# wthanone/kmerLSH

Hardware: AMD Instinct MI355X
Metric: k-mers·iterations/sec (LSH+cluster loop), 10M k-mers × 64 samples (higher is better)
Workload: dtype f32

## Files before the change

### kmerlsh_amd/csrc/klsh_ctx.h

```cpp
#pragma once
#include <hip/hip_runtime.h>
#include <stdint.h>
#include <stdio.h>
#include <string.h>

#include <atomic>
#include <chrono>
#include <cmath>
#include <string>
#include <thread>
#include <utility>
#include <vector>

#include "klsh.h"
#include "klsh_comm.h"
#include "klsh_internal.h"

extern "C" void klsh_host_hyperplanes(uint32_t base, uint64_t k0, uint64_t count, int d,
                                      int stride, float* out, int threads);

namespace klsh {

int fail(int code, const std::string& msg);
inline int set_error(int code, const char* msg) { return fail(code, msg); }
// ... 154 lines not shown
  uint32_t* pub_seq_dev = nullptr;
  uint32_t pub_seq = 0;
  static constexpr int kRing = 2 * 32;
  Counters* ring_host = nullptr;
  Counters* ring_dev = nullptr;
  bool ctr_clean = false;
  uint32_t* n_next_dev = nullptr;
  klsh::QueuedProjection spec;
  bool take_queued_projection() {
    const bool queued = spec.pending;
    if (queued && spec.swap) std::swap(keys, keys2);
    drop_queued_projection();
    return queued;
  }
  void drop_queued_projection() { spec.pending = spec.swap = false; }
  bool zero_copy = true;
  klsh::RunCounters* rc = nullptr;
  uint16_t* xh_alloc = nullptr;
  bool shadow_wanted(int d_) const {
    return pw.variant != klsh::kProjPacked && klsh::shadow_width_ok(d_);
  }
  bool tail_batch = true;
  bool tail_local = true;
  int last_hash_kernel = klsh::kPkNone;
  int last_hash_variant = klsh::kPvNone;
  uint64_t last_hash_close = 0;
  bool result_device = false;
  uint32_t result_rounds = 0;
  int64_t result_rank_us = 0;
  klsh::KmcHooks kmc;
  klsh::KcountHooks kcount;

  ~klsh_ctx() { release(); }

  bool phase_timing = false;

  uint64_t shard_min_rows = 1u << 21;
  uint32_t huge_quiet = 0;
  bool huge_fold_always = false;
  double comm_timeout_s = 600.0;

  int stop_after = 0;
  hipEvent_t counts_ev = nullptr;
  int progress = 0;
  void tick(int it) const {
    if (progress > 0 && it % progress == 0) {
// ... 37 lines not shown
```

### kmerlsh_amd/csrc/klsh_device.h

```cpp
#pragma once
#include <hip/hip_runtime.h>

#include "klsh_internal.h"

namespace klsh {
__device__ __forceinline__ unsigned long long stamp_now() { return __builtin_amdgcn_s_memrealtime(); }
__device__ __forceinline__ void kt_begin(const KTime& kt, int c) {
  if (kt.blk && threadIdx.x == 0) {
    const unsigned long long now = stamp_now();
    atomicMin(&kt.blk->set[kt.set].t0[c][blockIdx.x % kStampSlots].v, now);
    if (kt.phase >= 0) atomicMin(&kt.blk->set[kt.set].t0[kt.phase][blockIdx.x % kStampSlots].v, now);
  }
}
__device__ __forceinline__ void kt_end(const KTime& kt, int c) {
  if (kt.blk && threadIdx.x == 0) {
    const unsigned long long now = stamp_now();
    atomicMax(&kt.blk->set[kt.set].t1[c][blockIdx.x % kStampSlots].v, now);
    if (kt.phase >= 0) atomicMax(&kt.blk->set[kt.set].t1[kt.phase][blockIdx.x % kStampSlots].v, now);
  }
}
__device__ __forceinline__ void kt_fold_set(KStampBlock* blk, int f, uint32_t t) {
  if (t >= (uint32_t)KC_COUNT) return;
  KStampSet& st = blk->set[f];
  unsigned long long lo = ~0ull, hi = 0ull;
  for (int q = 0; q < kStampSlots; ++q) {
    lo = min(lo, __hip_atomic_load(&st.t0[t][q].v, __ATOMIC_RELAXED, __HIP_MEMORY_SCOPE_AGENT));
    hi = max(hi, __hip_atomic_load(&st.t1[t][q].v, __ATOMIC_RELAXED, __HIP_MEMORY_SCOPE_AGENT));
    __hip_atomic_store(&st.t0[t][q].v, ~0ull, __ATOMIC_RELAXED, __HIP_MEMORY_SCOPE_AGENT);
    __hip_atomic_store(&st.t1[t][q].v, 0ull, __ATOMIC_RELAXED, __HIP_MEMORY_SCOPE_AGENT);
  }
  if (hi != 0ull && lo != ~0ull && hi >= lo) {
// ... 362 lines not shown
```

### kmerlsh_amd/csrc/klsh_internal.h

```cpp
#pragma once

#include <hip/hip_ext.h>
#include <hip/hip_runtime_api.h>
#include <stdint.h>
#include <stdio.h>

#include <vector>

#include "klsh.h"

namespace klsh {

constexpr uint32_t kInvalid = 0xFFFFFFFFu;
constexpr uint32_t kNil = 0xFFFFFFFFu;
constexpr int kMaxHyperplanes = 32;
constexpr int kScanTile = 4096;
uint64_t sort_ws_words(uint64_t slots);
constexpr uint32_t kScanStatusWord = 64;
constexpr uint64_t kScanSumsWord = kScanStatusWord + 2ull * (1ull << 20);
inline uint64_t scan_ws_words(uint64_t slots) {
  return kScanSumsWord + (256 * slots) / kScanTile + 1024;
}

constexpr int kBigClasses = 4;
// ... 35 lines not shown
  KC_TAIL, KC_COMPACT, KC_SCREEN,
  KC_MERGE,
  KC_COUNT
};
constexpr int kStampSlots = 16;
struct alignas(128) StampLine {
  unsigned long long v;
  unsigned long long pad_[15];
};
struct KStampSet {
  StampLine t0[KC_COUNT][kStampSlots];
  StampLine t1[KC_COUNT][kStampSlots];
};
struct KStampBlock {
  KStampSet set[2];
  unsigned long long ticks[KC_COUNT];
  unsigned long long launches[KC_COUNT];
};
struct KTime {
  KStampBlock* blk;
  int set;
  int fold;
  int phase = -1;
};
constexpr KTime kNoTime{nullptr, 0, -1, -1};

struct MergeWork {
  uint2* cls[kGroupClasses];
  uint2* act[kGroupClasses];
  uint32_t screened;
  uint2* big[kBigClasses];
  uint2* huge;
  uint2* over;
  uint32_t* tile_sums;
  RunCounters* rc;
  uint32_t* run_ws;
  uint32_t* dlist;
  uint32_t* mark;
  uint32_t stamp;
  uint32_t big896_aux;
  uint32_t huge_cap;
  uint32_t huge_fold;
  uint64_t* long_P;
  uint32_t long_groups;
  uint32_t long_off = 4;
  uint32_t small_grid;
// ... 88 lines not shown

const uint32_t* radix_sort_top(const uint32_t* k0, const uint32_t* v0, uint32_t* k1, uint32_t* v1,
                               uint32_t n, int bits, uint32_t* ws, hipStream_t s, KTime kt,
                               const uint32_t* n_dev);
void launch_tail_local(const uint32_t* kin, const uint32_t* vin, uint32_t* kout, uint32_t* vout,
                       const uint32_t* dtot, int bits, int bucket_thr, const MergeWork& w,
                       hipStream_t s);
constexpr int kTailTopBits = 9;
constexpr int kTailLowBits = 19 - kTailTopBits > 10 ? 19 - kTailTopBits : 10;
inline bool tail_local_ok(uint32_t n_max, int bits) {
  return n_max <= (1u << 20) && bits > kTailTopBits && bits <= kTailTopBits + kTailLowBits;
}

constexpr int kRunListCount = kGroupClasses + kBigClasses + 2;
void launch_runs(const uint32_t* key, uint32_t lo, uint32_t n, int bucket_thr, const MergeWork& w,
                 hipStream_t s, const uint32_t* n_dev = nullptr);

struct Publish {
  Counters* host;
  uint32_t* seq_host;
  uint32_t seq;
  uint32_t* n_next;
  uint32_t* woff = nullptr;
};

struct LookBack {
  unsigned long long* status;
  mutable uint32_t epoch;
};

void launch_compact(const uint32_t* slots, uint32_t n, uint32_t* out, uint32_t* tile_sums,
                    Counters* ctr, hipStream_t s, const Publish* pub = nullptr,
                    RunCounters* rc = nullptr, KTime kt = kNoTime,
                    const LookBack* lb = nullptr, const uint32_t* n_dev = nullptr);
void launch_stamp_fold(KStampBlock* blk, int set, hipStream_t s);
void launch_publish_words(const uint32_t* a, uint32_t na, const uint32_t* b, uint32_t nb,
                          uint32_t* dst, uint32_t* seq_host, uint32_t seq, hipStream_t s);

void launch_convert(const Rows& r, const uint16_t* counts, uint32_t bs, const float* lut,
                    const float* v_kmers, uint32_t* keep, uint32_t* order, uint32_t* tile_sums,
                    Counters* ctr, hipStream_t s);

void launch_norms(const Rows& r, uint32_t n, hipStream_t s);
void launch_shadow_build(const Rows& r, uint64_t n, hipStream_t s);


// ... 149 lines not shown
```

### kmerlsh_amd/csrc/klsh_kernels.hip

```cpp
#include <hip/hip_runtime.h>

#include <stdlib.h>

#include <string>
#include <type_traits>

#include "klsh_device.h"

namespace klsh {

typedef float f32x2 __attribute__((ext_vector_type(2)));


__device__ __forceinline__ void pk_mac_lo(f32x2& acc, f32x2 w, f32x2 x) {
  f32x2 t;
  asm("v_pk_mul_f32 %1, %2, %3 op_sel_hi:[1,0]\n\tv_pk_add_f32 %0, %0, %1"
      : "+v"(acc), "=&v"(t) : "v"(w), "v"(x));
}
__device__ __forceinline__ void pk_mac_hi(f32x2& acc, f32x2 w, f32x2 x) {
  f32x2 t;
  asm("v_pk_mul_f32 %1, %2, %3 op_sel:[0,1] op_sel_hi:[1,1]\n\tv_pk_add_f32 %0, %0, %1"
      : "+v"(acc), "=&v"(t) : "v"(w), "v"(x));
}

// ... 849 lines not shown
    case 64: go_pk(k_project_pk<64, 2, 1>); break;
    default: {
      const size_t lds = sizeof(float4) * (size_t)r.dp * (size_t)((h + 3) / 4);
      if (lds <= 64 * 1024) {
        static const bool lds_ok =
            hipFuncSetAttribute(reinterpret_cast<const void*>(&k_project_wide_pk<1>),
                                hipFuncAttributeMaxDynamicSharedMemorySize, 64 * 1024) == hipSuccess;
        (void)lds_ok;
        k_project_wide_pk<1><<<grid, block, lds, s>>>(r.x, r.d, r.dp, slots, keys, n, W, h, key_or,
                                                      kt);
        pv = kPvWidePk;
      } else {
        pv = kPvGeneric;
        k_project_generic<<<grid, block, 0, s>>>(r.x, r.d, r.dp, slots, keys, n, W, h, key_or, kt);
      }
    }
  }
  return kPkPacked;
}

constexpr int kCompactTile = 4096;
__global__ __launch_bounds__(256) void k_compact_count(const uint32_t* __restrict__ slots,
                                                       uint32_t n, uint32_t* __restrict__ counts,
                                                       KTime kt) {
  __shared__ uint32_t wsum[4];
  kt_begin(kt, KC_COMPACT);
  const uint32_t t = threadIdx.x, lane = t & 63u, wv = t >> 6;
  const uint32_t T0 = blockIdx.x * (uint32_t)kCompactTile;
  uint32_t c = 0;
#pragma unroll
  for (int k = 0; k < kCompactTile / 256; ++k) {
    const uint32_t i = T0 + k * 256u + t;
    const uint32_t v = slots[i < n ? i : 0u];
    c += (uint32_t)__popcll(__ballot(i < n && v != kInvalid));
  }
  if (lane == 0) wsum[wv] = c;
  __syncthreads();
  if (t == 0) counts[blockIdx.x] = wsum[0] + wsum[1] + wsum[2] + wsum[3];
}

__device__ __forceinline__ void collect_run_counts(Counters* ctr, RunCounters* rc) {
  if (!rc) return;
  ctr->n_seg = rc->n_seg.v;
  rc->n_seg.v = 0u;
#pragma unroll
  for (int c = 0; c < kGroupClasses; ++c) {
    ctr->n_cls[c] = rc->n_cls[c].v;
    rc->n_cls[c].v = 0u;
  }
#pragma unroll
// ... 6 lines not shown
  ctr->n_over = rc->n_over.v;
  rc->n_over.v = 0u;
  ctr->n_small_rows = rc->n_small_rows.v;
  rc->n_small_rows.v = 0u;
#pragma unroll
  for (int c = 0; c < kBigClasses; ++c) {
    ctr->n_big_rows[c] = rc->n_big_rows[c].v;
    rc->n_big_rows[c].v = 0u;
  }
  ctr->n_huge_rows = rc->n_huge_rows.v;
  rc->n_huge_rows.v = 0u;
#pragma unroll
  for (int c = 0; c < kGroupClasses; ++c) rc->n_act[c].v = 0u;
  ctr->n_act_rows = rc->n_act_rows.v;
  rc->n_act_rows.v = 0u;
  ctr->screened = rc->screened.v;
  rc->screened.v = 0u;
}

__device__ __forceinline__ void publish_counters(Counters* ctr, uint32_t total, const Publish& pub,
                                                 uint32_t n_in) {
  Counters c = *ctr;
  c.total = total;
  if (pub.n_next) *pub.n_next = total;
  if (pub.woff && n_in) *pub.woff += 31u - (uint32_t)__builtin_clz(n_in);
  const uint32_t* src = reinterpret_cast<const uint32_t*>(&c);
  uint32_t* dst = reinterpret_cast<uint32_t*>(pub.host);
  for (int i = 0; i < (int)(sizeof(Counters) / 4); ++i) {
    __hip_atomic_store(dst + i, src[i], __ATOMIC_RELAXED, __HIP_MEMORY_SCOPE_SYSTEM);
    reinterpret_cast<uint32_t*>(ctr)[i] = 0u;
  }
  __threadfence_system();
  __hip_atomic_store(pub.seq_host, pub.seq, __ATOMIC_RELEASE, __HIP_MEMORY_SCOPE_SYSTEM);
}

__global__ void k_publish(Counters* ctr, Publish pub, RunCounters* rc) {
  collect_run_counts(ctr, rc);
  if (pub.host) publish_counters(ctr, ctr->total, pub, 0u);
}

__global__ __launch_bounds__(256) void k_compact_apply(const uint32_t* __restrict__ slots,
                                                       uint32_t n,
                                                       const uint32_t* __restrict__ counts,
                                                       uint32_t* __restrict__ out,
                                                       uint32_t* __restrict__ total,
                                                       Counters* ctr, Publish pub,
                                                       RunCounters* rc, KTime kt) {
  constexpr int K = kCompactTile / 256;
  __shared__ uint32_t cnt[K * 4], pre[K * 4 + 1], wsum[4];
  const uint32_t t = threadIdx.x, lane = t & 63u, wv = t >> 6;
  const uint32_t T0 = blockIdx.x * (uint32_t)kCompactTile;
  uint32_t before = 0;
  for (uint32_t j = t; j < blockIdx.x; j += 256) before += counts[j];
#pragma unroll
  for (int o = 32; o > 0; o >>= 1) before += __shfl_xor(before, o, 64);
  if (lane == 0) wsum[wv] = before;
  uint32_t v[K];
  uint64_t m[K];
#pragma unroll
  for (int k = 0; k < K; ++k) {
    const uint32_t i = T0 + k * 256u + t;
    v[k] = slots[i < n ? i : 0u];
  }
#pragma unroll
  for (int k = 0; k < K; ++k) {
    if (T0 + k * 256u + t >= n) v[k] = kInvalid;
    m[k] = __ballot(v[k] != kInvalid);
    if (lane == 0) cnt[k * 4 + wv] = (uint32_t)__popcll(m[k]);
  }
  __syncthreads();
  if (t == 0) {
    uint32_t a = wsum[0] + wsum[1] + wsum[2] + wsum[3];
    for (int q = 0; q < K * 4; ++q) {
// ... 74 lines not shown
      a += cnt[q];
    }
    pre[K * 4] = a;
  }
  __syncthreads();
  const uint64_t below = lane ? (~0ull >> (64 - lane)) : 0ull;
#pragma unroll
  for (int k = 0; k < K; ++k)
    if (v[k] != kInvalid) out[pre[k * 4 + wv] + (uint32_t)__popcll(m[k] & below)] = v[k];
  if (blockIdx.x == gridDim.x - 1 && t == 0) {
    *total = pre[K * 4];
    collect_run_counts(ctr, rc);
    if (pub.host) publish_counters(ctr, pre[K * 4], pub, n);
  }
  kt_end(kt, KC_COMPACT);
}

void launch_compact(const uint32_t* slots, uint32_t n, uint32_t* out, uint32_t* tile_sums,
                    Counters* ctr, hipStream_t s, const Publish* pub, RunCounters* rc, KTime kt,
                    const LookBack* lb, const uint32_t* n_dev) {
  const Publish none{nullptr, nullptr, 0u, nullptr};
  if (n_dev) {
    const uint32_t ntiles = (n + kCompactTile - 1) / kCompactTile;
    if (!lb || !lb->status || ntiles == 0 || ntiles > 256u) return;
    const uint32_t epoch = ++lb->epoch;
    k_compact_lb<<<ntiles, 256, 0, s>>>(slots, n, out, lb->status, epoch, &ctr->total, ctr,
                                        pub ? *pub : none, rc, kt, n_dev);
    return;
  }
  if (n == 0) {
    (void)hipMemsetAsync(&ctr->total, 0, sizeof(uint32_t), s);
    k_publish<<<1, 1, 0, s>>>(ctr, pub ? *pub : none, rc);
    return;
  }
  const uint32_t ntiles = (n + kCompactTile - 1) / kCompactTile;
  if (lb && lb->status && ntiles <= 256u) {
    const uint32_t epoch = ++lb->epoch;
    k_compact_lb<<<ntiles, 256, 0, s>>>(slots, n, out, lb->status, epoch, &ctr->total, ctr,
                                        pub ? *pub : none, rc, kt, nullptr);
    return;
  }
  uint32_t* counts = tile_sums + kScanSumsWord;
  k_compact_count<<<ntiles, 256, 0, s>>>(slots, n, counts, kt);
  k_compact_apply<<<ntiles, 256, 0, s>>>(slots, n, counts, out, &ctr->total, ctr, pub ? *pub : none,
                                         rc, kt);
}

__global__ __launch_bounds__(256) void k_convert(Rows r, const uint16_t* __restrict__ counts,
                                                 uint32_t bs, const float* __restrict__ lut,
                                                 const float* __restrict__ v_kmers,
                                                 uint32_t* __restrict__ keep) {
  const uint32_t i = blockIdx.x * 256u + threadIdx.x;
  if (i >= bs) return;
  const int d = r.d;
  float* x = r.x + (size_t)i * r.dp;
  uint64_t total = 0;
  float nn = 0.0f;
  for (int j = 0; j < d; ++j) {
    const uint32_t c = counts[(size_t)j * bs + i];
    total += c;
    const float v = lut[c] - v_kmers[j];
    x[j] = v;
    nn = nn + v * v;
  }
  for (int j = d; j < r.dp; ++j) x[j] = 0.0f;
  r.nrm[i] = nn;
  r.cnt[i] = 1;
  r.head[i] = i;
// ... 77 lines not shown
```

### kmerlsh_amd/csrc/klsh_loop.cpp

```cpp
#include <stddef.h>
#include <stdlib.h>
#include <string.h>

#include <algorithm>
#include <deque>

#include "klsh_loop.h"

namespace klsh {

static void count_class_rows(klsh_stats* st, const Counters& c, uint64_t n, bool tail) {
  uint64_t big_rows = 0, big_runs = 0, small_runs = 0;
  for (int b = 0; b < kBigClasses; ++b) big_rows += c.n_big_rows[b], big_runs += c.n_big[b];
  for (int b = 0; b < kGroupClasses; ++b) small_runs += c.n_cls[b];
  for (int k : {KC_PROJECT, KC_SORT, KC_COMPACT}) st->kern[k].rows += n;
  st->kern[KC_RUNS].rows += n;
  st->kern[KC_RUNS].runs += c.n_seg;
  st->kern[KC_HUGE].rows += c.n_huge_rows;
  st->kern[KC_HUGE].runs += c.n_huge;
  if (c.screened) {
    st->kern[KC_SCREEN].rows += c.n_small_rows;
    st->kern[KC_SCREEN].runs += small_runs;
  }
  const uint64_t merged_small = c.screened ? c.n_act_rows : c.n_small_rows;
// ... 167 lines not shown
    const uint64_t k = *rng_counter;
    *rng_counter += (uint64_t)h2;
    if (st) {
      st->hyperplanes += (uint64_t)h2;
      st->nested_calls += 1;
    }
    if (int e = ctx->ensure_hyperplanes(seed_base, k, (uint64_t)h2, st ? &st->host_ms : nullptr))
      return e;
    const uint32_t key_or = 0x80000000u | ((oi & 1u) << 30);
    launch_project(ctx->rows, fv + p, ctx->nk1, b, ctx->hyperplane_ptr(k), h2, key_or, s, &ctx->pw);
    uint32_t *rk = nullptr, *rv = nullptr;
    radix_sort(ctx->nk1, fv + p, ctx->nk2, ctx->nv2, b, h2, ctx->hist, &rk, &rv, s);
    KLSH_HIP(hipMemcpyAsync(fk + p, rk, 4ull * b, hipMemcpyDeviceToDevice, s));
    if (rv != fv + p) KLSH_HIP(hipMemcpyAsync(fv + p, rv, 4ull * b, hipMemcpyDeviceToDevice, s));
    KLSH_HIP(hipMemsetAsync(ctx->rc, 0, sizeof(RunCounters), s));
    launch_merge(ctx->rows, fk, fv, p, p + b, thr, -1, ctx->mw, ctx->ctr, s);
    KLSH_HIP(hipGetLastError());
  }
  launch_compact(fv, n, out, ctx->tile_sums, ctx->ctr, s, nullptr, ctx->rc);
  KLSH_HIP(hipGetLastError());
  return ctx->sync_counters();
}

int merge_and_compact(klsh_ctx* ctx, uint32_t* fk, uint32_t* fv, uint32_t n, float thr,
                      int bucket_thr, uint32_t seed_base, uint64_t* rng_counter, klsh_stats* st,
                      bool timed, const std::function<int(uint32_t*)>* after, KTime kt) {
  uint32_t* out = (fv == ctx->order) ? ctx->alt : ctx->order;
  if (int e = merge_main(ctx, fk, fv, n, thr, bucket_thr, out, st, timed, true, after, kt))
    return e;
  ctx->mw.big896_aux = ctx->h_ctr->n_big[kBigClasses - 1] >= 64u ? 1u : 0u;
  ctx->mw.huge_cap = ctx->h_ctr->n_huge == 0 ? 64u : 0u;
  ctx->huge_quiet = ctx->h_ctr->n_huge == 0 ? ctx->huge_quiet + 1 : 0;
  ctx->mw.huge_fold = (ctx->huge_quiet >= 4 || ctx->huge_fold_always) ? 1u : 0u;
  if (ctx->h_ctr->n_over > 0) {
    std::vector<uint2> over;
    uint64_t hyp = 0;
    if (int e = oversize_runs(ctx, &over, &hyp)) return e;
    if (int e = merge_nested(ctx, fk, fv, n, thr, over, seed_base, rng_counter, out, st))
      return e;
  }
  if (out == ctx->alt) std::swap(ctx->order, ctx->alt);
  ctx->n_live = ctx->h_ctr->total;
  return 0;
}

static bool batch_eligible(const klsh_ctx* ctx, uint64_t n, int bucket_thr, int iters_left) {
  if (!ctx->tail_batch || n < 2 || n >= std::min<uint64_t>(tail_merge_max(ctx->mw), 1u << 20) ||
      iters_left < 2)
    return false;
  if (bucket_thr >= 0 && n > (uint64_t)bucket_thr) return false;
  if (!ctx->zero_copy || !ctx->ring_dev || !ctx->lb.status || ctx->phase_timing) return false;
  if (!project_device_n_ok(ctx->d) || ctx->mw.dlist) return false;
  if (diag_host_driven()) return false;
  return (uint64_t)iters_left * (uint64_t)floor_log2(n) * (uint64_t)ctx->dp <= (64ull << 20);
}

static int run_batched(klsh_ctx* ctx, float& threshold, float sim_step, int it, int it_end,
                       int bucket_size_threshold, uint32_t seed_base, uint64_t* rng_counter,
                       uint64_t* nt_trace, klsh_stats* st,
                       const std::function<KTime(uint64_t)>& ktime) {
  hipStream_t s = ctx->stream;
#ifdef KLSH_MERGE_PROF
  if (getenv("KLSH_MERGE_PROF")) {
    fprintf(stderr, "[mprof] ---- head: iterations before %d\n", it);
    merge_prof_dump(stderr);
    fprintf(stderr, "[mprof] ---- tail: iterations %d..%d\n", it, it_end - 1);
  }
#endif
  constexpr int C = klsh_ctx::kRing / 2;
  uint64_t n_known = ctx->n_live;
  const int h0 = floor_log2(n_known);
  const uint64_t k0 = *rng_counter;
  const uint64_t need = (uint64_t)(it_end - it) * (uint64_t)h0;
  if (!(ctx->W && ctx->w_base == seed_base && ctx->w_dp == ctx->dp && ctx->w_d == ctx->d &&
        k0 >= ctx->w_k0 && k0 + need <= ctx->w_k0 + ctx->w_count)) {
    if (!ctx->lazy_covers(seed_base, k0, need)) KLSH_HIP(hipStreamSynchronize(s));
    if (int e = ctx->ensure_hyperplanes(seed_base, k0, need, &st->host_ms)) return e;
  }
  uint32_t* n_dev = ctx->n_next_dev;
  uint32_t* woff_dev = ctx->n_next_dev + 1;
  KLSH_HIP(hipMemsetD32Async(n_dev, (int)(uint32_t)n_known, 1, s));
  KLSH_HIP(hipMemsetD32Async(woff_dev, (int)(uint32_t)(k0 - ctx->w_k0), 1, s));
  const uint64_t queued_k = ctx->spec.k;
  bool queued = ctx->take_queued_projection();
  if (!queued && !ctx->ctr_clean)
    if (int e = ctx->reset_counters()) return e;
  if (queued && queued_k != k0) return fail(KLSH_E_STATE, "queued projection out of step");

  struct Chunk {
    int it0, count, slot0;
    uint32_t seq_last;
  };
  std::deque<Chunk> inflight;
  int next = it, slot = 0;
  float thr = threshold;
  uint64_t n_max = n_known;
  auto enqueue = [&](int count) -> int {
    const int hb = floor_log2(n_max);
    for (int c = 0; c < count; ++c, ++next) {
      const KTime kt = ktime(ctx->kt_iter++);
      if (!queued)
        launch_project_device_n(ctx->rows, ctx->order, ctx->keys, (uint32_t)n_max, ctx->W, n_dev, s,
                                kt, woff_dev, &ctx->pw);
      queued = false;
      uint32_t *fk = nullptr, *fv = nullptr;
      const bool local = ctx->tail_local && tail_local_ok((uint32_t)n_max, hb);
      LaunchScope launch(ctx->mw, kt);
      if (local) {
        const uint32_t* dtot = radix_sort_top(ctx->keys, ctx->order, ctx->keys2, ctx->alt,
                                              (uint32_t)n_max, hb, ctx->hist, s, kt, n_dev);
        launch_tail_local(ctx->keys2, ctx->alt, ctx->keys, ctx->order, dtot, hb,
                          bucket_size_threshold, ctx->mw, s);
        fk = ctx->keys;
        fv = ctx->order;
      } else {
        radix_sort(ctx->keys, ctx->order, ctx->keys2, ctx->alt, (uint32_t)n_max, hb, ctx->hist,
                   &fk, &fv, s, kt, n_dev);
      }
      launch_merge(ctx->rows, fk, fv, 0, (uint32_t)n_max, thr, bucket_size_threshold, ctx->mw,
                   ctx->ctr, s, n_dev, local);
      uint32_t* out = (fv == ctx->order) ? ctx->alt : ctx->order;
      Publish pub{ctx->ring_dev + slot, ctx->pub_seq_dev, ++ctx->pub_seq, n_dev, woff_dev};
      launch_compact(fv, (uint32_t)n_max, out, ctx->tile_sums, ctx->ctr, s, &pub, ctx->rc, kt,
                     &ctx->lb, n_dev);
      if (out == ctx->alt) std::swap(ctx->order, ctx->alt);
      thr -= sim_step;
      slot = (slot + 1) % klsh_ctx::kRing;
    }
    KLSH_HIP(hipGetLastError());
    return 0;
  };
  while (next < it_end || !inflight.empty()) {
    while (next < it_end && inflight.size() < 2) {
      const Chunk ch{next, std::min(C, it_end - next), slot, 0u};
      if (int e = enqueue(ch.count)) return e;
      inflight.push_back(ch);
      inflight.back().seq_last = ctx->pub_seq;
    }
    const Chunk ch = inflight.front();
    inflight.pop_front();
    if (int e = ctx->wait_seq(ch.seq_last)) return e;
    for (int c = 0; c < ch.count; ++c) {
      const Counters cc = ctx->ring_host[(ch.slot0 + c) % klsh_ctx::kRing];
      const uint64_t n_in = n_known;
      if (cc.err)
        return fail(KLSH_E_HIP, "device protocol failure (look-back wait limit), code " +
                                    std::to_string(cc.err));
      if (cc.n_over || n_in == 0 || cc.total == 0 || cc.total > n_in)
        return fail(KLSH_E_STATE, "queued iteration published inconsistent counters");
      const int h = floor_log2(n_in);
      if (nt_trace) nt_trace[ch.it0 + c] = n_in;
      ctx->tick(ch.it0 + c);
      *rng_counter += (uint64_t)h;
      account_iteration(st, n_in, h, cc.total);
      if (ctx->kernel_timing && ctx->kstamp) count_class_rows(st, cc, n_in, true);
      diag_log_batched(ch.it0 + c, n_in, h, cc);
      *ctx->h_ctr = cc;
      n_known = cc.total;
    }
    n_max = n_known;
  }
  threshold = thr;
  ctx->n_live = n_known;
  ctx->ctr_clean = true;
  return 0;
}

int run_single(klsh_ctx* ctx, float& threshold, float sim_step, int it_begin, int it_end,
               int bucket_size_threshold, uint32_t seed_base, uint64_t* rng_counter,
               uint64_t* nt_trace, klsh_stats* st) {
  hipStream_t s = ctx->stream;
  const uint64_t kt_first = ctx->kt_iter;
  auto ktime = [&](uint64_t j) -> KTime {
    if (!ctx->kernel_timing || !st) return kNoTime;
    if (!ctx->kstamp) return kNoTime;
    return KTime{ctx->kstamp, (int)(j & 1u), j > kt_first ? (int)((j - 1) & 1u) : -1};
  };
  for (int it = it_begin; it < it_end; ++it) {
    const uint64_t n = ctx->n_live;
    if (batch_eligible(ctx, n, bucket_size_threshold, it_end - it)) {
      const std::function<KTime(uint64_t)> kt_fn = ktime;
      if (int e = run_batched(ctx, threshold, sim_step, it, it_end, bucket_size_threshold,
                              seed_base, rng_counter, nt_trace, st, kt_fn))
        return e;
      break;
    }
    const double t_it = diag_iter_begin();
    if (nt_trace) nt_trace[it] = n;
    ctx->tick(it);
    if (n == 0) {
      account_iteration(st, 0, 0, 0);
      threshold -= sim_step;
      continue;
    }
    const int h = floor_log2(n);
    const uint64_t k = *rng_counter;
    *rng_counter += (uint64_t)h;
    if (int e = ctx->ensure_hyperplanes(seed_base, k, (uint64_t)h, &st->host_ms)) return e;

    const QueuedProjection spec = ctx->spec;
    const bool queued = ctx->take_queued_projection();
    const uint64_t j = ctx->kt_iter++;
    if (queued && spec.k != k) return fail(KLSH_E_STATE, "queued projection out of step");
    const int pair = queued ? spec.pair : 0;
    const bool rec = ctx->hip_events || ctx->phase_timing;
    if (!queued) {
      if (!ctx->ctr_clean) if (int e = ctx->reset_counters()) return e;
      if (rec) KLSH_HIP(hipEventRecord(ctx->project_begin(pair), s));
      launch_project(ctx->rows, ctx->order, ctx->keys, (uint32_t)n, ctx->hyperplane_ptr(k), h, 0u,
// ... 24 lines not shown
      ctx->spec = QueuedProjection{true, k_next, next_pair, spec_out == ctx->keys2};
      return 0;
    };
    if (int e = merge_and_compact(ctx, fk, fv, (uint32_t)n, threshold, bucket_size_threshold,
                                  seed_base, rng_counter, st, ctx->phase_timing,
                                  ahead ? &queue_next : nullptr, ktime(j)))
      return e;
    if (ctx->spec.pending && *rng_counter != ctx->spec.k) {
      ctx->drop_queued_projection();
      if (ctx->kernel_timing && ctx->kstamp) {
        KStampSet* set = &ctx->kstamp->set[ctx->kt_iter & 1u];
        KLSH_HIP(hipMemsetAsync(&set->t0[KC_PROJECT][0], 0xFF, sizeof(set->t0[KC_PROJECT]), s));
        KLSH_HIP(hipMemsetAsync(&set->t1[KC_PROJECT][0], 0, sizeof(set->t1[KC_PROJECT]), s));
      }
    }
    if (rec) {
      st->project_ms += elapsed(ctx->project_begin(pair), ctx->project_end(pair));
      st->project_timed_launches += 1;
    }
    if (rec && ctx->phase_timing)
      st->sort_ms += elapsed(ctx->project_end(pair), ctx->ev[EV_SORT_END]);
    account_iteration(st, n, h, ctx->n_live);
    threshold -= sim_step;
    diag_log_iteration(ctx, it, n, h, t_it);
  }
  if (ctx->kernel_timing && ctx->kstamp && st && ctx->kt_iter > kt_first)
    if (int e = collect_kernel_times(ctx, (int)((ctx->kt_iter - 1) & 1u), st)) return e;
  return 0;
}

}

using namespace klsh;

extern "C" int klsh_cluster(klsh_ctx* ctx, float min_similarity, int iterations,
                            int bucket_size_threshold, uint32_t seed_base, uint64_t* rng_counter,
                            uint64_t* nt_trace, klsh_stats* stats) {
  if (!ctx || !rng_counter) return fail(KLSH_E_ARG, "null argument");
  if (!ctx->loaded) {
    if (ctx->comm) ctx->comm->abort();
    return fail(KLSH_E_STATE, "klsh_cluster before a load");
  }
  KLSH_HIP(hipSetDevice(ctx->device));
  if (stats && stats->struct_size != sizeof(klsh_stats))
    return fail(KLSH_E_ARG, "klsh_stats.struct_size != sizeof(klsh_stats): built against another "
                            "klsh.h (KLSH_ABI_VERSION " + std::to_string(KLSH_ABI_VERSION) + ")");
  klsh_stats local{};
  klsh_stats* st = stats ? stats : &local;
  memset(st, 0, sizeof(*st));
  st->struct_size = sizeof(*st);
  st->world = (uint64_t)ctx->world();
  ctx->mw.huge_cap = 0;
  ctx->mw.huge_fold = ctx->huge_fold_always ? 1u : 0u;
  ctx->huge_quiet = 0;
  const int run_iters = ctx->stop_after > 0 ? std::min(iterations, ctx->stop_after) : iterations;
  if (ctx->comm)
    return cluster_sharded(ctx, min_similarity, iterations, run_iters, bucket_size_threshold,
                           seed_base, rng_counter, nt_trace, st);
  const double t_start = now_ms();

  const float max_similarity = 0.95f;
  const float sim_step = (max_similarity - min_similarity) / (float)iterations;
  float threshold = max_similarity;

  ctx->ctr_clean = false;
  ctx->drop_queued_projection();
  ctx->mw.big896_aux = ctx->n_live >= (1u << 24) ? 1u : 0u;
  ctx->w_count = 0;
  if (ctx->n_live > 0 && iterations > 0) {
    if (int e = ctx->predraw_hyperplanes(seed_base, *rng_counter,
                                         (uint64_t)floor_log2(ctx->n_live), iterations,
                                         &st->host_ms))
      return e;
  }

  if (int e = run_single(ctx, threshold, sim_step, 0, run_iters, bucket_size_threshold, seed_base,
                         rng_counter, nt_trace, st))
// ... 17 lines not shown
```

### kmerlsh_amd/csrc/klsh_loop.h

```cpp
#pragma once
#include <functional>
#include <vector>

#include "klsh_ctx.h"

namespace klsh {

struct LaunchScope {
  MergeWork& mw;
  LaunchScope(MergeWork& w, KTime kt, hipEvent_t e0 = nullptr, hipEvent_t e1 = nullptr) : mw(w) {
    mw.kt = kt, mw.small_ev[0] = e0, mw.small_ev[1] = e1;
  }
  ~LaunchScope() { mw.kt = kNoTime, mw.small_ev[0] = mw.small_ev[1] = nullptr; }
  LaunchScope(const LaunchScope&) = delete;
};

struct DeltaScope {
  MergeWork& mw;
  DeltaScope(MergeWork& w, uint32_t* dlist, uint32_t* mark, uint32_t stamp) : mw(w) {
    mw.dlist = dlist, mw.mark = mark, mw.stamp = stamp;
  }
  ~DeltaScope() { mw.dlist = mw.mark = nullptr; }
  DeltaScope(const DeltaScope&) = delete;
};

inline void account_iteration(klsh_stats* st, uint64_t n, int h, uint64_t n_next) {
  st->iterations += 1;
  if (n == 0) return;
  st->hyperplanes += (uint64_t)h;
  st->project_launches += 1;
  st->sum_rows += n;
  st->sum_proj_bits += n * (uint64_t)h;
  st->sum_merges += n - n_next;
}

int merge_main(klsh_ctx* ctx, uint32_t* fk, uint32_t* fv, uint32_t n, float thr, int bucket_thr,
               uint32_t* out, klsh_stats* st, bool timed, bool sync = true,
               const std::function<int(uint32_t*)>* after = nullptr, KTime kt = kNoTime);
int oversize_runs(klsh_ctx* ctx, std::vector<uint2>* over, uint64_t* hyperplanes);
int merge_nested(klsh_ctx* ctx, uint32_t* fk, uint32_t* fv, uint32_t n, float thr,
                 const std::vector<uint2>& over, uint32_t seed_base, uint64_t* rng_counter,
                 uint32_t* out, klsh_stats* st);
int merge_and_compact(klsh_ctx* ctx, uint32_t* fk, uint32_t* fv, uint32_t n, float thr,
                      int bucket_thr, uint32_t seed_base, uint64_t* rng_counter, klsh_stats* st,
                      bool timed, const std::function<int(uint32_t*)>* after = nullptr,
                      KTime kt = kNoTime);
int run_single(klsh_ctx* ctx, float& threshold, float sim_step, int it_begin, int it_end,
               int bucket_size_threshold, uint32_t seed_base, uint64_t* rng_counter,
               uint64_t* nt_trace, klsh_stats* st);
int cluster_sharded(klsh_ctx* ctx, float min_similarity, int iterations, int run_iters,
                    int bucket_size_threshold, uint32_t seed_base, uint64_t* rng_counter,
                    uint64_t* nt_trace, klsh_stats* st);

}
```

### kmerlsh_amd/csrc/klsh_merge.hip

```cpp
#include <algorithm>
#include <cstdlib>
#include <cstring>
#include <limits>

#include "klsh_merge_common.h"
#include "klsh_merge_small.h"
#include "klsh_merge_runs.h"
#include "klsh_merge_gram.h"
#include "klsh_merge_huge.h"
#include "klsh_merge_big.h"
#include "klsh_merge_long.h"
#include "klsh_merge_wide.h"

namespace klsh {

static float sim_roundtrip(float s) {
  volatile float dist = 1.0f - s;
  volatile float sim = 1.0f - dist;
  return sim;
}
static uint32_t ordered(float f) {
  uint32_t u;
  memcpy(&u, &f, 4);
  return (u & 0x80000000u) ? ~u : (u | 0x80000000u);
// ... 234 lines not shown
  else group(k_merge_group_wide<32>, 4, 2, dc);
  if (gram && gmin <= 16) group(k_merge_group_wide<16, 512>, 3, 4, dg);
  else group(k_merge_group_wide<16>, 3, 4, dc);
  if (gram && gmin <= 8) group(k_merge_group_wide<8, 512>, 2, 8, dg);
  else group(k_merge_group_wide<8>, 2, 8, dc);
  group(k_merge_group_wide<4>, 1, 16, dc);
  group(k_merge_group_wide<2>, 0, 32, dc);
}

void launch_runs(const uint32_t* key, uint32_t lo, uint32_t n, int bucket_thr, const MergeWork& w,
                 hipStream_t s, const uint32_t* n_dev) {
  const uint32_t ntiles = (n + kRunTile - 1) / kRunTile;
  uint32_t* counts = w.run_ws;
  uint32_t* tail_ends = counts + (size_t)kRunRows * ntiles;
  uint2* heads_fl = reinterpret_cast<uint2*>(counts + (((kRunRows + 1u) * ntiles + 1u) & ~1u));
  uint64_t* hbits = reinterpret_cast<uint64_t*>(heads_fl + ntiles);
  k_runs_count<<<ntiles, 256, 0, s>>>(key, lo, n, bucket_thr, ntiles, hbits, heads_fl, counts,
                                      w.kt, n_dev);
  const bool fused = ntiles <= 256u;
  if (fused) {
    k_runs_write<true><<<ntiles, 256, 0, s>>>(lo, n, bucket_thr, ntiles, hbits, heads_fl,
                                              tail_ends, counts, w, n_dev);
  } else {
    k_runs_scan<<<kRunRows, 256, 0, s>>>(counts, ntiles, n, bucket_thr, heads_fl, tail_ends, w.rc);
    k_runs_write<false><<<ntiles, 256, 0, s>>>(lo, n, bucket_thr, ntiles, hbits, heads_fl,
                                               tail_ends, counts, w, nullptr);
  }
}

void launch_tail_local(const uint32_t* kin, const uint32_t* vin, uint32_t* kout, uint32_t* vout,
                       const uint32_t* dtot, int bits, int bucket_thr, const MergeWork& w,
                       hipStream_t s) {
  k_tail_local<<<1u << kTailTopBits, 256, 0, s>>>(kin, vin, kout, vout, dtot, bits - kTailTopBits,
                                                   bucket_thr, w);
}

void launch_merge(const Rows& r, const uint32_t* key, uint32_t* slots, uint32_t lo, uint32_t hi,
                  float thr, int bucket_thr, const MergeWork& w, Counters* ctr, hipStream_t s,
                  const uint32_t* n_dev, bool runs_ready) {
  if (hi <= lo) return;
  const uint32_t n = hi - lo;
  if (n_dev && (lo != 0 || n >= tail_merge_max(w))) return;
  const Decider dc = make_decider(thr);
  if (!runs_ready) launch_runs(key, lo, n, bucket_thr, w, s, n_dev);
  MergeWork wm = w;
  if (w.kt.blk && (n >= tail_merge_max(w) || !project_device_n_ok(r.d))) wm.kt.phase = KC_MERGE;
  switch (r.d) {
// ... 64 lines not shown
```

### kmerlsh_amd/csrc/klsh_merge_runs.h

```cpp
#pragma once

#include "klsh_merge_common.h"

namespace klsh {

constexpr uint32_t kRunTile = 4096;
constexpr int kRunLists = kGroupClasses + kBigClasses + 2;
constexpr int kRunRows = kRunLists + 2 + kBigClasses + 1;

__device__ __forceinline__ uint32_t* run_counter(RunCounters* rc, int l) {
  return l < kGroupClasses ? &rc->n_cls[l].v
         : l < kGroupClasses + kBigClasses ? &rc->n_big[l - kGroupClasses].v
         : l == kRunLists - 2 ? &rc->n_huge.v
         : l == kRunLists - 1 ? &rc->n_over.v
         : l == kRunLists ? &rc->n_seg.v
         : l == kRunLists + 1 ? &rc->n_small_rows.v
         : l < kRunLists + 2 + kBigClasses ? &rc->n_big_rows[l - kRunLists - 2].v
                                           : &rc->n_huge_rows.v;
}

__device__ __forceinline__ int run_class(uint32_t b, int bucket_thr) {
  if (bucket_thr >= 0 && b > (uint32_t)bucket_thr) return kRunLists - 1;
  if (b > 64u) {
    if (b > (uint32_t)kBigRows[kBigClasses - 1]) return kRunLists - 2;
// ... 136 lines not shown
  for (int o = 32; o > 0; o >>= 1) {
    heads += __shfl_xor(heads, o, 64);
    small_rows += __shfl_xor(small_rows, o, 64);
#pragma unroll
    for (int c = 0; c <= kBigClasses; ++c) lrows[c] += __shfl_xor(lrows[c], o, 64);
  }
  if (lane == 0 && heads) atomicAdd(&lcnt[kRunLists], heads);
  if (lane == 0 && small_rows) atomicAdd(&lcnt[kRunLists + 1], small_rows);
#pragma unroll
  for (int c = 0; c <= kBigClasses; ++c)
    if (lane == 0 && lrows[c]) atomicAdd(&lcnt[kRunLists + 2 + c], lrows[c]);
  __syncthreads();
  if (t < (uint32_t)kRunRows) counts[(size_t)t * ntiles + blockIdx.x] = lcnt[t];
}

__device__ __forceinline__ uint32_t last_run_len(uint32_t j, uint32_t last, uint32_t tail_end) {
  return last == ~0u ? 0u : tail_end - (j * kRunTile + last);
}

__global__ __launch_bounds__(256) void k_runs_scan(uint32_t* __restrict__ counts, uint32_t ntiles,
                                                   uint32_t n, int bucket_thr,
                                                   const uint2* __restrict__ heads_fl,
                                                   uint32_t* __restrict__ tail_ends,
                                                   RunCounters* rc) {
  const int l = (int)blockIdx.x;
  uint32_t* row = counts + (size_t)l * ntiles;
  const uint32_t t = threadIdx.x;
  const uint32_t per = (ntiles + 255u) / 256u;
  const uint32_t a = min(ntiles, t * per), e = min(ntiles, a + per);
  constexpr uint32_t CH = 8;
  uint32_t fmin = ~0u;
  for (uint32_t i0 = a; i0 < e; i0 += CH) {
    uint32_t hx[CH];
#pragma unroll
    for (uint32_t c = 0; c < CH; ++c) hx[c] = heads_fl[min(i0 + c, e - 1u)].x;
#pragma unroll
    for (uint32_t c = 0; c < CH; ++c) fmin = min(fmin, hx[c]);
  }
  uint32_t after = block_excl_suffix_min_256(fmin);
  uint32_t acc = 0;
  for (uint32_t i1 = e; i1 > a;) {
    const uint32_t i0 = i1 - a > CH ? i1 - CH : a;
    uint2 hf[CH];
    uint32_t rv[CH];
#pragma unroll
    for (uint32_t c = 0; c < CH; ++c) {
      const uint32_t j = min(i0 + c, i1 - 1u);
      hf[c] = heads_fl[j];
// ... 313 lines not shown
```

### kmerlsh_amd/csrc/klsh_options.cpp

```cpp
#include <string.h>

#include "klsh_ctx.h"

namespace {

struct Option {
  const char* name;
  int64_t (*get)(klsh_ctx*);
  int (*set)(klsh_ctx*, int64_t);
};

int out_of_range(const char* name, const char* range) {
  return fail(KLSH_E_ARG, std::string(name) + " must be " + range);
}
int grid(const char* name, int64_t v) {
  return v < 0 || v > (1 << 20) ? out_of_range(name, "in [0, 2^20]") : 0;
}
int zero_or_one(const char* name, int64_t v) {
  return v != 0 && v != 1 ? out_of_range(name, "0 or 1") : 0;
}
int at_least_zero(const char* name, int64_t v) { return v < 0 ? out_of_range(name, ">= 0") : 0; }

#define GET(expr) [](klsh_ctx* c) -> int64_t { return (int64_t)(expr); }
#define SET(...) [](klsh_ctx* c, int64_t v) -> int { __VA_ARGS__ }
#define CHECKED(name, check, field, conv) \
  {name, GET(c->field), SET(if (int e = check(name, v)) return e; c->field = conv; return 0;)}
#define FLAG(name, field) {name, GET(c->field), SET(c->field = v != 0; return 0;)}
#define GRID(name, field) CHECKED(name, grid, field, (uint32_t)v)
#define BOOL01(name, field) CHECKED(name, zero_or_one, field, v != 0)
#define COUNT(name, field) CHECKED(name, at_least_zero, field, (uint64_t)v)
#define INVERTED01(name, field)  \
  {name, GET(c->field ? 0 : 1), \
   SET(if (int e = zero_or_one(name, v)) return e; c->field = v ? 0u : 1u; return 0;)}
#define READONLY(name, expr) {name, GET(expr), nullptr}

const Option kOptions[] = {
    COUNT("shard_min_rows", shard_min_rows),
    FLAG("phase_timing", phase_timing),
    FLAG("kernel_timing", kernel_timing),
    FLAG("tail_batch", tail_batch),
    FLAG("huge_fold", huge_fold_always),
    FLAG("tail_local", tail_local),
    BOOL01("result_device", result_device),
    BOOL01("hyperplane_async", hyperplane_async),
    COUNT("hyperplane_window", hyperplane_window),
    {"progress", GET(c->progress), SET(
        if (v < 0 || v > INT32_MAX) return out_of_range("progress", ">= 0");
        c->progress = (int)v;
        return 0;)},
    {"stop_after", GET(c->stop_after), SET(
        if (v < 0 || v > INT32_MAX) return out_of_range("stop_after", "in [0, 2^31)");
        c->stop_after = (int)v;
        return 0;)},
    {"projection", GET(c->pw.variant), SET(
        if (v != klsh::kProjAuto && v != klsh::kProjPacked)
          return out_of_range("projection", "0 (default) or 1 (exact packed chains)");
        KLSH_HIP(hipSetDevice(c->device));
        c->pw.variant = (uint32_t)v;
        return c->apply_projection_variant();)},
    {"wide_gram", GET(c->mw.wide_gram), SET(
        if (v != 0 && v != 8 && v != 16 && v != 32 && v != 64)
          return out_of_range("wide_gram", "0, 8, 16, 32 or 64");
        c->mw.wide_gram = (uint32_t)v;
// ... 106 lines not shown
```

Before: 28.23 billion.

## Allow device-queued iterations to halt on oversize runs and fall back to host

```diff
diff --git a/kmerlsh_amd/csrc/klsh_ctx.h b/kmerlsh_amd/csrc/klsh_ctx.h
--- a/kmerlsh_amd/csrc/klsh_ctx.h
+++ b/kmerlsh_amd/csrc/klsh_ctx.h
@@ -200,6 +200,11 @@
   }
   bool tail_batch = true;
   bool tail_local = true;
+  uint32_t queue_rows = 0;
+  uint32_t queue_chunk = 0;
+  static constexpr uint32_t kQueueRows = 1u << 20;
+  static constexpr int kBandChunk = 8;
+  uint64_t queued_iterations = 0, queued_halts = 0;
   int last_hash_kernel = klsh::kPkNone;
   int last_hash_variant = klsh::kPvNone;
   uint64_t last_hash_close = 0;
diff --git a/kmerlsh_amd/csrc/klsh_device.h b/kmerlsh_amd/csrc/klsh_device.h
--- a/kmerlsh_amd/csrc/klsh_device.h
+++ b/kmerlsh_amd/csrc/klsh_device.h
@@ -6,7 +6,7 @@
 namespace klsh {
 __device__ __forceinline__ unsigned long long stamp_now() { return __builtin_amdgcn_s_memrealtime(); }
 __device__ __forceinline__ void kt_begin(const KTime& kt, int c) {
-  if (kt.blk && threadIdx.x == 0) {
+  if (kt.blk && threadIdx.x == 0 && (!kt.n_dev || *kt.n_dev != 0u)) {
     const unsigned long long now = stamp_now();
     atomicMin(&kt.blk->set[kt.set].t0[c][blockIdx.x % kStampSlots].v, now);
     if (kt.phase >= 0) atomicMin(&kt.blk->set[kt.set].t0[kt.phase][blockIdx.x % kStampSlots].v, now);
diff --git a/kmerlsh_amd/csrc/klsh_internal.h b/kmerlsh_amd/csrc/klsh_internal.h
--- a/kmerlsh_amd/csrc/klsh_internal.h
+++ b/kmerlsh_amd/csrc/klsh_internal.h
@@ -81,6 +81,7 @@
   int set;
   int fold;
   int phase = -1;
+  const uint32_t* n_dev = nullptr;
 };
 constexpr KTime kNoTime{nullptr, 0, -1, -1};
 
@@ -215,6 +216,7 @@
   uint32_t seq;
   uint32_t* n_next;
   uint32_t* woff = nullptr;
+  uint32_t halt = 0;
 };
 
 struct LookBack {
diff --git a/kmerlsh_amd/csrc/klsh_kernels.hip b/kmerlsh_amd/csrc/klsh_kernels.hip
--- a/kmerlsh_amd/csrc/klsh_kernels.hip
+++ b/kmerlsh_amd/csrc/klsh_kernels.hip
@@ -895,10 +895,15 @@
 constexpr int kCompactTile = 4096;
 __global__ __launch_bounds__(256) void k_compact_count(const uint32_t* __restrict__ slots,
                                                        uint32_t n, uint32_t* __restrict__ counts,
-                                                       KTime kt) {
+                                                       KTime kt, const uint32_t* __restrict__ n_dev,
+                                                       uint32_t* __restrict__ n_snap) {
   __shared__ uint32_t wsum[4];
   kt_begin(kt, KC_COMPACT);
   const uint32_t t = threadIdx.x, lane = t & 63u, wv = t >> 6;
+  if (n_dev) {
+    n = *n_dev;
+    if (blockIdx.x == 0 && t == 0) *n_snap = n;
+  }
   const uint32_t T0 = blockIdx.x * (uint32_t)kCompactTile;
   uint32_t c = 0;
 #pragma unroll
@@ -951,8 +956,9 @@
                                                  uint32_t n_in) {
   Counters c = *ctr;
   c.total = total;
-  if (pub.n_next) *pub.n_next = total;
-  if (pub.woff && n_in) *pub.woff += 31u - (uint32_t)__builtin_clz(n_in);
+  const bool halt = pub.halt && c.n_over != 0u;
+  if (pub.n_next) *pub.n_next = halt ? 0u : total;
+  if (pub.woff && n_in && !halt) *pub.woff += 31u - (uint32_t)__builtin_clz(n_in);
   const uint32_t* src = reinterpret_cast<const uint32_t*>(&c);
   uint32_t* dst = reinterpret_cast<uint32_t*>(pub.host);
   for (int i = 0; i < (int)(sizeof(Counters) / 4); ++i) {
@@ -974,10 +980,12 @@
                                                        uint32_t* __restrict__ out,
                                                        uint32_t* __restrict__ total,
                                                        Counters* ctr, Publish pub,
-                                                       RunCounters* rc, KTime kt) {
+                                                       RunCounters* rc, KTime kt,
+                                                       const uint32_t* __restrict__ n_snap) {
   constexpr int K = kCompactTile / 256;
   __shared__ uint32_t cnt[K * 4], pre[K * 4 + 1], wsum[4];
   const uint32_t t = threadIdx.x, lane = t & 63u, wv = t >> 6;
+  if (n_snap) n = *n_snap;
   const uint32_t T0 = blockIdx.x * (uint32_t)kCompactTile;
   uint32_t before = 0;
   for (uint32_t j = t; j < blockIdx.x; j += 256) before += counts[j];
@@ -1098,7 +1106,15 @@
   const Publish none{nullptr, nullptr, 0u, nullptr};
   if (n_dev) {
     const uint32_t ntiles = (n + kCompactTile - 1) / kCompactTile;
-    if (!lb || !lb->status || ntiles == 0 || ntiles > 256u) return;
+    if (!lb || !lb->status || ntiles == 0) return;
+    if (ntiles > 256u) {
+      uint32_t* counts = tile_sums + kScanSumsWord;
+      uint32_t* n_snap = counts + ntiles;
+      k_compact_count<<<ntiles, 256, 0, s>>>(slots, n, counts, kt, n_dev, n_snap);
+      k_compact_apply<<<ntiles, 256, 0, s>>>(slots, n, counts, out, &ctr->total, ctr,
+                                             pub ? *pub : none, rc, kt, n_snap);
+      return;
+    }
     const uint32_t epoch = ++lb->epoch;
     k_compact_lb<<<ntiles, 256, 0, s>>>(slots, n, out, lb->status, epoch, &ctr->total, ctr,
                                         pub ? *pub : none, rc, kt, n_dev);
@@ -1117,9 +1133,9 @@
     return;
   }
   uint32_t* counts = tile_sums + kScanSumsWord;
-  k_compact_count<<<ntiles, 256, 0, s>>>(slots, n, counts, kt);
+  k_compact_count<<<ntiles, 256, 0, s>>>(slots, n, counts, kt, nullptr, nullptr);
   k_compact_apply<<<ntiles, 256, 0, s>>>(slots, n, counts, out, &ctr->total, ctr, pub ? *pub : none,
-                                         rc, kt);
+                                         rc, kt, nullptr);
 }
 
 __global__ __launch_bounds__(256) void k_convert(Rows r, const uint16_t* __restrict__ counts,
diff --git a/kmerlsh_amd/csrc/klsh_loop.cpp b/kmerlsh_amd/csrc/klsh_loop.cpp
--- a/kmerlsh_amd/csrc/klsh_loop.cpp
+++ b/kmerlsh_amd/csrc/klsh_loop.cpp
@@ -213,33 +213,40 @@
   return ctx->sync_counters();
 }
 
+static void note_run_counts(klsh_ctx* ctx) {
+  ctx->mw.big896_aux = ctx->h_ctr->n_big[kBigClasses - 1] >= 64u ? 1u : 0u;
+  ctx->mw.huge_cap = ctx->h_ctr->n_huge == 0 ? 64u : 0u;
+  ctx->huge_quiet = ctx->h_ctr->n_huge == 0 ? ctx->huge_quiet + 1 : 0;
+  ctx->mw.huge_fold = (ctx->huge_quiet >= 4 || ctx->huge_fold_always) ? 1u : 0u;
+}
+
+int finish_oversize(klsh_ctx* ctx, uint32_t* fk, uint32_t* fv, uint32_t n, float thr,
+                    uint32_t seed_base, uint64_t* rng_counter, uint32_t* out, klsh_stats* st) {
+  if (ctx->h_ctr->n_over == 0) return 0;
+  std::vector<uint2> over;
+  uint64_t hyp = 0;
+  if (int e = oversize_runs(ctx, &over, &hyp)) return e;
+  return merge_nested(ctx, fk, fv, n, thr, over, seed_base, rng_counter, out, st);
+}
+
 int merge_and_compact(klsh_ctx* ctx, uint32_t* fk, uint32_t* fv, uint32_t n, float thr,
                       int bucket_thr, uint32_t seed_base, uint64_t* rng_counter, klsh_stats* st,
                       bool timed, const std::function<int(uint32_t*)>* after, KTime kt) {
   uint32_t* out = (fv == ctx->order) ? ctx->alt : ctx->order;
   if (int e = merge_main(ctx, fk, fv, n, thr, bucket_thr, out, st, timed, true, after, kt))
     return e;
-  ctx->mw.big896_aux = ctx->h_ctr->n_big[kBigClasses - 1] >= 64u ? 1u : 0u;
-  ctx->mw.huge_cap = ctx->h_ctr->n_huge == 0 ? 64u : 0u;
-  ctx->huge_quiet = ctx->h_ctr->n_huge == 0 ? ctx->huge_quiet + 1 : 0;
-  ctx->mw.huge_fold = (ctx->huge_quiet >= 4 || ctx->huge_fold_always) ? 1u : 0u;
-  if (ctx->h_ctr->n_over > 0) {
-    std::vector<uint2> over;
-    uint64_t hyp = 0;
-    if (int e = oversize_runs(ctx, &over, &hyp)) return e;
-    if (int e = merge_nested(ctx, fk, fv, n, thr, over, seed_base, rng_counter, out, st))
-      return e;
-  }
+  note_run_counts(ctx);
+  if (int e = finish_oversize(ctx, fk, fv, n, thr, seed_base, rng_counter, out, st)) return e;
   if (out == ctx->alt) std::swap(ctx->order, ctx->alt);
   ctx->n_live = ctx->h_ctr->total;
   return 0;
 }
 
 static bool batch_eligible(const klsh_ctx* ctx, uint64_t n, int bucket_thr, int iters_left) {
-  if (!ctx->tail_batch || n < 2 || n >= std::min<uint64_t>(tail_merge_max(ctx->mw), 1u << 20) ||
-      iters_left < 2)
+  const uint32_t rows = ctx->queue_rows ? ctx->queue_rows : klsh_ctx::kQueueRows;
+  if (!ctx->tail_batch || n < 2 || n >= std::min(tail_merge_max(ctx->mw), rows) || iters_left < 2)
     return false;
-  if (bucket_thr >= 0 && n > (uint64_t)bucket_thr) return false;
+  if (rows == (1u << 20) && bucket_thr >= 0 && n > (uint64_t)bucket_thr) return false;
   if (!ctx->zero_copy || !ctx->ring_dev || !ctx->lb.status || ctx->phase_timing) return false;
   if (!project_device_n_ok(ctx->d) || ctx->mw.dlist) return false;
   if (diag_host_driven()) return false;
@@ -249,7 +256,7 @@
 static int run_batched(klsh_ctx* ctx, float& threshold, float sim_step, int it, int it_end,
                        int bucket_size_threshold, uint32_t seed_base, uint64_t* rng_counter,
                        uint64_t* nt_trace, klsh_stats* st,
-                       const std::function<KTime(uint64_t)>& ktime) {
+                       const std::function<KTime(uint64_t)>& ktime, int* it_next) {
   hipStream_t s = ctx->stream;
 #ifdef KLSH_MERGE_PROF
   if (getenv("KLSH_MERGE_PROF")) {
@@ -259,6 +266,7 @@
   }
 #endif
   constexpr int C = klsh_ctx::kRing / 2;
+  const int c_band = ctx->queue_chunk ? (int)ctx->queue_chunk : klsh_ctx::kBandChunk;
   uint64_t n_known = ctx->n_live;
   const int h0 = floor_log2(n_known);
   const uint64_t k0 = *rng_counter;
@@ -282,6 +290,12 @@
     int it0, count, slot0;
     uint32_t seq_last;
   };
+  struct Enqueued {
+    uint32_t *fk, *fv, *out, *order, *alt;
+    uint64_t kt_iter;
+    float thr;
+  };
+  std::vector<Enqueued> enq;
   std::deque<Chunk> inflight;
   int next = it, slot = 0;
   float thr = threshold;
@@ -289,7 +303,8 @@
   auto enqueue = [&](int count) -> int {
     const int hb = floor_log2(n_max);
     for (int c = 0; c < count; ++c, ++next) {
-      const KTime kt = ktime(ctx->kt_iter++);
+      KTime kt = ktime(ctx->kt_iter++);
+      kt.n_dev = n_dev;
       if (!queued)
         launch_project_device_n(ctx->rows, ctx->order, ctx->keys, (uint32_t)n_max, ctx->W, n_dev, s,
                                 kt, woff_dev, &ctx->pw);
@@ -311,10 +326,11 @@
       launch_merge(ctx->rows, fk, fv, 0, (uint32_t)n_max, thr, bucket_size_threshold, ctx->mw,
                    ctx->ctr, s, n_dev, local);
       uint32_t* out = (fv == ctx->order) ? ctx->alt : ctx->order;
-      Publish pub{ctx->ring_dev + slot, ctx->pub_seq_dev, ++ctx->pub_seq, n_dev, woff_dev};
+      Publish pub{ctx->ring_dev + slot, ctx->pub_seq_dev, ++ctx->pub_seq, n_dev, woff_dev, 1u};
       launch_compact(fv, (uint32_t)n_max, out, ctx->tile_sums, ctx->ctr, s, &pub, ctx->rc, kt,
                      &ctx->lb, n_dev);
       if (out == ctx->alt) std::swap(ctx->order, ctx->alt);
+      enq.push_back(Enqueued{fk, fv, out, ctx->order, ctx->alt, ctx->kt_iter, thr});
       thr -= sim_step;
       slot = (slot + 1) % klsh_ctx::kRing;
     }
@@ -323,7 +339,7 @@
   };
   while (next < it_end || !inflight.empty()) {
     while (next < it_end && inflight.size() < 2) {
-      const Chunk ch{next, std::min(C, it_end - next), slot, 0u};
+      const Chunk ch{next, std::min(n_max >= (1u << 20) ? c_band : C, it_end - next), slot, 0u};
       if (int e = enqueue(ch.count)) return e;
       inflight.push_back(ch);
       inflight.back().seq_last = ctx->pub_seq;
@@ -337,12 +353,39 @@
       if (cc.err)
         return fail(KLSH_E_HIP, "device protocol failure (look-back wait limit), code " +
                                     std::to_string(cc.err));
-      if (cc.n_over || n_in == 0 || cc.total == 0 || cc.total > n_in)
+      if (n_in == 0 || cc.total == 0 || cc.total > n_in)
         return fail(KLSH_E_STATE, "queued iteration published inconsistent counters");
       const int h = floor_log2(n_in);
       if (nt_trace) nt_trace[ch.it0 + c] = n_in;
       ctx->tick(ch.it0 + c);
       *rng_counter += (uint64_t)h;
+      ctx->queued_iterations += 1;
+      if (cc.n_over) {
+        const int t = ch.it0 + c;
+        if (int e = ctx->wait_seq(ctx->pub_seq)) return e;
+        for (int v = t + 1; v < next; ++v) {
+          const Counters vc = ctx->ring_host[(ch.slot0 + c + (v - t)) % klsh_ctx::kRing];
+          if (vc.err || vc.total || vc.n_seg || vc.n_over)
+            return fail(KLSH_E_STATE, "queued iteration published inconsistent counters");
+        }
+        const Enqueued& q = enq[(size_t)(t - it)];
+        if (ctx->kernel_timing && ctx->kstamp) count_class_rows(st, cc, n_in, true);
+        diag_log_batched(t, n_in, h, cc);
+        *ctx->h_ctr = cc;
+        note_run_counts(ctx);
+        ctx->order = q.order, ctx->alt = q.alt;
+        ctx->kt_iter = q.kt_iter;
+        ctx->ctr_clean = true;
+        ctx->queued_halts += 1;
+        if (int e = finish_oversize(ctx, q.fk, q.fv, (uint32_t)n_in, q.thr, seed_base, rng_counter,
+                                    q.out, st))
+          return e;
+        ctx->n_live = ctx->h_ctr->total;
+        account_iteration(st, n_in, h, ctx->n_live);
+        threshold = q.thr - sim_step;
+        *it_next = t + 1;
+        return 0;
+      }
       account_iteration(st, n_in, h, cc.total);
       if (ctx->kernel_timing && ctx->kstamp) count_class_rows(st, cc, n_in, true);
       diag_log_batched(ch.it0 + c, n_in, h, cc);
@@ -354,6 +397,7 @@
   threshold = thr;
   ctx->n_live = n_known;
   ctx->ctr_clean = true;
+  *it_next = it_end;
   return 0;
 }
 
@@ -367,15 +411,21 @@
     if (!ctx->kstamp) return kNoTime;
     return KTime{ctx->kstamp, (int)(j & 1u), j > kt_first ? (int)((j - 1) & 1u) : -1};
   };
+  bool hold = false;
   for (int it = it_begin; it < it_end; ++it) {
     const uint64_t n = ctx->n_live;
-    if (batch_eligible(ctx, n, bucket_size_threshold, it_end - it)) {
+    if (!hold && batch_eligible(ctx, n, bucket_size_threshold, it_end - it)) {
       const std::function<KTime(uint64_t)> kt_fn = ktime;
+      int it_next = it_end;
       if (int e = run_batched(ctx, threshold, sim_step, it, it_end, bucket_size_threshold,
-                              seed_base, rng_counter, nt_trace, st, kt_fn))
+                              seed_base, rng_counter, nt_trace, st, kt_fn, &it_next))
         return e;
-      break;
-    }
+      if (it_next >= it_end) break;
+      hold = true;
+      it = it_next - 1;
+      continue;
+    }
+    const uint64_t nested_before = st->nested_calls;
     const double t_it = diag_iter_begin();
     if (nt_trace) nt_trace[it] = n;
     ctx->tick(it);
@@ -446,6 +496,7 @@
       st->sort_ms += elapsed(ctx->project_end(pair), ctx->ev[EV_SORT_END]);
     account_iteration(st, n, h, ctx->n_live);
     threshold -= sim_step;
+    hold = st->nested_calls != nested_before;
     diag_log_iteration(ctx, it, n, h, t_it);
   }
   if (ctx->kernel_timing && ctx->kstamp && st && ctx->kt_iter > kt_first)
@@ -477,6 +528,7 @@
   ctx->mw.huge_cap = 0;
   ctx->mw.huge_fold = ctx->huge_fold_always ? 1u : 0u;
   ctx->huge_quiet = 0;
+  ctx->queued_iterations = ctx->queued_halts = 0;
   const int run_iters = ctx->stop_after > 0 ? std::min(iterations, ctx->stop_after) : iterations;
   if (ctx->comm)
     return cluster_sharded(ctx, min_similarity, iterations, run_iters, bucket_size_threshold,
diff --git a/kmerlsh_amd/csrc/klsh_loop.h b/kmerlsh_amd/csrc/klsh_loop.h
--- a/kmerlsh_amd/csrc/klsh_loop.h
+++ b/kmerlsh_amd/csrc/klsh_loop.h
@@ -41,6 +41,8 @@
 int merge_nested(klsh_ctx* ctx, uint32_t* fk, uint32_t* fv, uint32_t n, float thr,
                  const std::vector<uint2>& over, uint32_t seed_base, uint64_t* rng_counter,
                  uint32_t* out, klsh_stats* st);
+int finish_oversize(klsh_ctx* ctx, uint32_t* fk, uint32_t* fv, uint32_t n, float thr,
+                    uint32_t seed_base, uint64_t* rng_counter, uint32_t* out, klsh_stats* st);
 int merge_and_compact(klsh_ctx* ctx, uint32_t* fk, uint32_t* fv, uint32_t n, float thr,
                       int bucket_thr, uint32_t seed_base, uint64_t* rng_counter, klsh_stats* st,
                       bool timed, const std::function<int(uint32_t*)>* after = nullptr,
diff --git a/kmerlsh_amd/csrc/klsh_merge.hip b/kmerlsh_amd/csrc/klsh_merge.hip
--- a/kmerlsh_amd/csrc/klsh_merge.hip
+++ b/kmerlsh_amd/csrc/klsh_merge.hip
@@ -280,7 +280,8 @@
     k_runs_write<true><<<ntiles, 256, 0, s>>>(lo, n, bucket_thr, ntiles, hbits, heads_fl,
                                               tail_ends, counts, w, n_dev);
   } else {
-    k_runs_scan<<<kRunRows, 256, 0, s>>>(counts, ntiles, n, bucket_thr, heads_fl, tail_ends, w.rc);
+    k_runs_scan<<<kRunRows, 256, 0, s>>>(counts, ntiles, n, bucket_thr, heads_fl, tail_ends, w.rc,
+                                         n_dev);
     k_runs_write<false><<<ntiles, 256, 0, s>>>(lo, n, bucket_thr, ntiles, hbits, heads_fl,
                                                tail_ends, counts, w, nullptr);
   }
diff --git a/kmerlsh_amd/csrc/klsh_merge_runs.h b/kmerlsh_amd/csrc/klsh_merge_runs.h
--- a/kmerlsh_amd/csrc/klsh_merge_runs.h
+++ b/kmerlsh_amd/csrc/klsh_merge_runs.h
@@ -182,8 +182,10 @@
                                                    uint32_t n, int bucket_thr,
                                                    const uint2* __restrict__ heads_fl,
                                                    uint32_t* __restrict__ tail_ends,
-                                                   RunCounters* rc) {
+                                                   RunCounters* rc,
+                                                   const uint32_t* __restrict__ n_dev) {
   const int l = (int)blockIdx.x;
+  if (n_dev) n = *n_dev;
   uint32_t* row = counts + (size_t)l * ntiles;
   const uint32_t t = threadIdx.x;
   const uint32_t per = (ntiles + 255u) / 256u;
diff --git a/kmerlsh_amd/csrc/klsh_options.cpp b/kmerlsh_amd/csrc/klsh_options.cpp
--- a/kmerlsh_amd/csrc/klsh_options.cpp
+++ b/kmerlsh_amd/csrc/klsh_options.cpp
@@ -39,6 +39,16 @@
     FLAG("phase_timing", phase_timing),
     FLAG("kernel_timing", kernel_timing),
     FLAG("tail_batch", tail_batch),
+    {"queue_rows", GET(c->queue_rows ? c->queue_rows : klsh_ctx::kQueueRows), SET(
+        if (v < 0 || v > (1 << 22)) return out_of_range("queue_rows", "in [0, 2^22]");
+        c->queue_rows = (uint32_t)v;
+        return 0;)},
+    {"queue_chunk", GET(c->queue_chunk ? c->queue_chunk : klsh_ctx::kBandChunk), SET(
+        if (v < 0 || v > klsh_ctx::kRing / 2) return out_of_range("queue_chunk", "in [0, 32]");
+        c->queue_chunk = (uint32_t)v;
+        return 0;)},
+    READONLY("queued_iterations", c->queued_iterations),
+    READONLY("queued_halts", c->queued_halts),
     FLAG("huge_fold", huge_fold_always),
     FLAG("tail_local", tail_local),
     BOOL01("result_device", result_device),
```

After: 27.63 billion. 2.1% lower.
